# zixunh/vipe

Measured on AMD Instinct MI355X. Metric: dense-BA+flow update iters/s, 512x384 48-KF graph, higher is better.
Workload: dtype f16 (correlation, GRU; fp32 accumulate) + f32 geometry/BA (fp64 reduced system)

## Files before the change

### vipe_amd/csrc/ba.hip

```cpp
#include <stdlib.h>

#include "term_geom.cuh"

namespace {

#include "ba_common.cuh"
#include "ba_plan.inc"
#include "ba_accumulate.inc"
#include "ba_solve_band.inc"
#include "ba_solve_dense.inc"
#include "ba_solve_global.inc"
#include "ba_retract.inc"

hipEvent_t overlap_event() {
  static thread_local hipEvent_t ev[64] = {};
  int d = 0;
  (void)hipGetDevice(&d);
  hipEvent_t& e = ev[d & 63];
  if (!e && hipEventCreateWithFlags(&e, hipEventDisableTiming) != hipSuccess) e = nullptr;
  return e;
}

int overlap_piece(const vipe_ba_params& p, hipEvent_t ev, int piece, int n_pieces, bool gated) {
  hipStream_t side = (hipStream_t)p.overlap_stream;
  if (gated && ev && hipStreamWaitEvent(side, ev, 0) != hipSuccess) return VIPE_EINVAL;
  return p.overlap_fn(p.overlap_user, piece, n_pieces, p.overlap_stream);
}

template <int CAM, int F>
int run_iters(const BAArgs& a, hipStream_t s, int* pieces_done) {
  const int tiles = (a.P + TILE - 1) / TILE;
  const size_t sbytes = sizeof(double) * (size_t)a.w.ld * a.w.ld;
  const size_t nmax = (size_t)a.w.ld - 1;
  const size_t fixed = ((sizeof(SolveLds) + 15) / 16) * 16;
  int panel_cap = (int)std::min<size_t>(nmax + 1, (150 * 1024 - fixed) / (NB * sizeof(double)));
  panel_cap = (panel_cap + 3) & ~3;
  const size_t solve_lds = fixed + (size_t)NB * panel_cap * sizeof(double);
  const size_t band_lds = 158 * 1024;
  static std::atomic<uint64_t> attr_set{0};
  vipe_once_per_device(attr_set, [] {
    (void)hipFuncSetAttribute((const void*)ba_solve_band_kernel, hipFuncAttributeMaxDynamicSharedMemorySize, 160 * 1024);
    (void)hipFuncSetAttribute((const void*)ba_solve_kernel, hipFuncAttributeMaxDynamicSharedMemorySize, 160 * 1024);
    (void)hipFuncSetAttribute((const void*)ba_solve_dense_kernel, hipFuncAttributeMaxDynamicSharedMemorySize, 160 * 1024);
    (void)hipFuncSetAttribute((const void*)chol_backsub_kernel, hipFuncAttributeMaxDynamicSharedMemorySize, 64 * 1024);
  });
  static std::atomic<uint64_t> tmpl_set{0};
  vipe_once_per_device(tmpl_set, [] {
    (void)hipFuncSetAttribute((const void*)ba_accum_mfma_kernel<CAM, F>, hipFuncAttributeMaxDynamicSharedMemorySize, (int)accum_mfma_lds());
    (void)hipFuncSetAttribute((const void*)ba_walk_kernel<CAM, F>, hipFuncAttributeMaxDynamicSharedMemorySize, (int)walk_lds());
    (void)hipFuncSetAttribute((const void*)ba_walk_rig_kernel<CAM, 4>, hipFuncAttributeMaxDynamicSharedMemorySize, (int)walk_rig_lds());
    (void)hipFuncSetAttribute((const void*)ba_walk_rig_kernel<CAM, RG_VMAX>, hipFuncAttributeMaxDynamicSharedMemorySize, (int)walk_rig_lds());
  });
  const bool retract_clears = !a.p.motion_only;
  const bool overlap = a.p.overlap_stream && a.p.overlap_fn;
  hipEvent_t ev = overlap ? overlap_event() : nullptr;
  for (int it = 0; it < a.p.n_iters; ++it) {
    if (!(retract_clears && (it > 0 || a.p.reuse_plan))) {
      hipError_t e1 = hipMemsetAsync(a.w.S, 0, sbytes, s);
      hipError_t e2 = hipMemsetAsync(a.w.Hd, 0, sizeof(double) * nmax, s);
      if (e1 != hipSuccess || e2 != hipSuccess) return (int)(e1 != hipSuccess ? e1 : e2);
    }
    if (a.mv) {
      if (a.p.n_views <= 4) ba_walk_rig_kernel<CAM, 4><<<dim3(tiles, a.nF), TILE, walk_rig_lds(), s>>>(a);
      else ba_walk_rig_kernel<CAM, RG_VMAX><<<dim3(tiles, a.nF), TILE, walk_rig_lds(), s>>>(a);
      ba_schur_kernel<0><<<dim3(SC_GRID, a.nF), TILE, 0, s>>>(a);
      if (ev && hipEventRecord(ev, s) != hipSuccess) return VIPE_EINVAL;
      ba_solve_kernel<<<1, SOLVE_T, solve_lds, s>>>(a, panel_cap);
      launch_tiled_cholesky(a, s);
      if (overlap) {
        const int rc = overlap_piece(a.p, ev, it, a.p.n_iters, true);
        if (rc != VIPE_OK) return rc;
        ++*pieces_done;
      }
      if (!a.p.motion_only) ba_retract_kernel<0><<<dim3(tiles, a.nF), TILE, 0, s>>>(a);
      continue;
    }
    const int hint = a.force_general ? 0 : a.p.path_hint;
    const bool prof = a.p.profile_ev0 && a.p.profile_ev1 &&
                      it == (a.p.profile_iter < 0 || a.p.profile_iter >= a.p.n_iters ? a.p.n_iters - 1 : a.p.profile_iter);
    if (prof && hipEventRecord((hipEvent_t)a.p.profile_ev0, s) != hipSuccess) return VIPE_EINVAL;
    if (!(hint & 2)) ba_accum_mfma_kernel<CAM, F><<<dim3(tiles, a.nF), TILE, accum_mfma_lds(), s>>>(a);
    if (!(hint & 1)) {
      ba_walk_kernel<CAM, F><<<dim3(tiles, a.nF), TILE, walk_lds(), s>>>(a);
      ba_schur_kernel<F><<<dim3(SC_GRID, a.nF), TILE, 0, s>>>(a);
    }
    if (prof && hipEventRecord((hipEvent_t)a.p.profile_ev1, s) != hipSuccess) return VIPE_EINVAL;
    if (ev && hipEventRecord(ev, s) != hipSuccess) return VIPE_EINVAL;
    if (!(hint & 8)) ba_solve_band_kernel<<<1, 2 * BAND_T, band_lds, s>>>(a, (int)(band_lds / sizeof(double)));
    if (!(hint & 16)) ba_solve_dense_kernel<<<1, DN_T, band_lds, s>>>(a, (int)(band_lds / sizeof(double)));
    if (!(hint & 4)) {
      ba_solve_kernel<<<1, SOLVE_T, solve_lds, s>>>(a, panel_cap);
      launch_tiled_cholesky(a, s);
    }
    if (overlap) {
      const int rc = overlap_piece(a.p, ev, it, a.p.n_iters, true);
      if (rc != VIPE_OK) return rc;
      ++*pieces_done;
    }
    if (!a.p.motion_only) ba_retract_kernel<F><<<dim3(tiles, a.nF), TILE, 0, s>>>(a);
  }
  return vipe_launch_status();
}

}

VIPE_EXPORT int64_t vipe_dense_ba_workspace_bytes(const vipe_ba_params* p) {
  if (!p || p->n_poses <= 0 || p->n_views <= 0 || p->ht <= 0 || p->wd <= 0 || p->M < 0) return VIPE_EINVAL;
  return (int64_t)carve(*p, nullptr, nullptr);
}

VIPE_EXPORT int vipe_dense_ba(const vipe_ba_params* p, float* d_poses, float* d_disps, const float* d_disps_sens,
                              float* d_intrinsics, float* d_rig, const float* d_target, const float* d_weight,
                              const float* d_disp_damping, const int64_t* d_pi, const int64_t* d_qi,
                              const int64_t* d_pj, const int64_t* d_qj, const int64_t* d_di, void* d_workspace,
                              int64_t workspace_bytes, int* d_info, void* stream) {
  VIPE_CHECK_ARG(p && d_poses && d_disps && d_disps_sens && d_intrinsics && d_rig && d_disp_damping && d_workspace);
  VIPE_CHECK_ARG(p->n_poses > 0 && p->n_views > 0 && p->ht > 0 && p->wd > 0 && p->M >= 0 && p->n_iters >= 0);
  VIPE_CHECK_ARG(p->t0 <= p->t1 && p->intr_factor > 0);
  VIPE_CHECK_ARG(p->camera == VIPE_CAM_PINHOLE || p->camera == VIPE_CAM_MEI);
  VIPE_CHECK_ARG(p->M == 0 || (d_target && d_weight && d_pi && d_qi && d_pj && d_qj && d_di));
  if (is_multiview(*p) && p->n_views > RG_VMAX) return VIPE_EUNSUPPORTED;
  if ((int64_t)p->n_poses * p->n_views > 65535) return VIPE_EINVAL;
  BAArgs a;
  a.p = *p;
  if ((int64_t)carve(*p, (char*)d_workspace, &a.w) > workspace_bytes) return VIPE_ENOSPACE;
  a.poses = d_poses; a.disps = d_disps; a.intr = d_intrinsics; a.rig = d_rig;
  a.sens = d_disps_sens; a.target = d_target; a.weight = d_weight; a.eta = d_disp_damping;
  a.pi = d_pi; a.qi = d_qi; a.pj = d_pj; a.qj = d_qj; a.di = d_di;
  a.P = p->ht * p->wd;
  a.nF = p->n_poses * p->n_views;
  a.D = p->camera == VIPE_CAM_MEI ? 1 : 0;
  a.mv = is_multiview(*p) ? 1 : 0;
  a.nintr = tail_intr(*p);
  a.ntail = a.nintr + tail_rig(*p);
  a.force_general = (p->solver_options & VIPE_BA_OPT_GENERAL_ACCUMULATE) != 0;
  a.band2 = !(p->solver_options & VIPE_BA_OPT_ONE_CHAIN);
  a.droid = 0;
  a.dz_out = nullptr;
  hipStream_t s = as_stream(stream);
  int rc = VIPE_OK, pieces_done = 0;
  if (p->M > 0 && p->n_iters > 0) {
    ba_sens_kernel<<<a.nF, 256, 0, s>>>(d_disps_sens, a.w.sens_sum, a.P, a.w.info);
    if (!p->reuse_plan) ba_plan_kernel<<<1, 1024, 0, s>>>(a);
    const int F = p->optimize_intrinsics ? 1 + a.D : 0;
    if (p->camera == VIPE_CAM_PINHOLE) rc = F ? run_iters<VIPE_CAM_PINHOLE, 1>(a, s, &pieces_done) : run_iters<VIPE_CAM_PINHOLE, 0>(a, s, &pieces_done);
    else rc = F ? run_iters<VIPE_CAM_MEI, 2>(a, s, &pieces_done) : run_iters<VIPE_CAM_MEI, 0>(a, s, &pieces_done);
    if (rc != VIPE_OK) return rc;
    if (d_info) {
      hipError_t e = hipMemcpyAsync(d_info, a.w.info, 8 * sizeof(int), hipMemcpyDeviceToDevice, s);
      if (e != hipSuccess) return (int)e;
    }
  }
  if (p->overlap_stream && p->overlap_fn) {
    const int n_pieces = p->n_iters > 0 ? p->n_iters : 1;
    for (; pieces_done < n_pieces; ++pieces_done) {
      rc = overlap_piece(*p, nullptr, pieces_done, n_pieces, false);
      if (rc != VIPE_OK) return rc;
    }
  }
  const int64_t nd = (int64_t)a.nF * a.P;
  clamp_min_kernel<<<(int)std::min<int64_t>((nd + 255) / 256, 2048), 256, 0, s>>>(d_disps, nd, 1e-3f);
  return vipe_launch_status();
}

namespace {
size_t droid_extra_bytes(int E) { return align_up(8 * (size_t)(E + 1)) + align_up(7 * 4); }
vipe_ba_params droid_params(int n_poses, int ht, int wd, int E, int t0, int t1, int iterations, float lm, float ep,
                            int motion_only) {
  vipe_ba_params p = {};
  p.n_poses = n_poses; p.n_views = 1; p.ht = ht; p.wd = wd; p.M = E; p.t0 = t0; p.t1 = t1; p.n_iters = iterations;
  p.pose_damping = lm; p.pose_ep = ep; p.motion_only = motion_only; p.limited_disp = 0; p.optimize_intrinsics = 0;
  p.optimize_rig_rotation = 0; p.camera = VIPE_CAM_PINHOLE; p.alpha = 0.05f; p.weight_scale = 0.001f; p.intr_factor = 1.0f;
  p.reuse_plan = 0; p.path_hint = 0;
  return p;
}
}

VIPE_EXPORT int64_t vipe_ba_workspace_bytes(int n_poses, int ht, int wd, int E) {
  if (n_poses <= 0 || ht <= 0 || wd <= 0 || E < 0) return VIPE_EINVAL;
  const vipe_ba_params p = droid_params(n_poses, ht, wd, E, 0, 0, 0, 0.f, 0.f, 0);
  return (int64_t)(carve(p, nullptr, nullptr) + droid_extra_bytes(E));
}

VIPE_EXPORT int vipe_ba(float* d_poses, float* d_disps, const float* d_intrinsics, const float* d_disps_sens,
                        const float* d_targets, const float* d_weights, const float* d_eta, const int64_t* d_ii,
                        const int64_t* d_jj, int n_poses, int ht, int wd, int E, int n_eta, int t0, int t1,
                        int iterations, float lm, float ep, int motion_only, float* d_dx, float* d_dz,
                        void* d_workspace, int64_t workspace_bytes, void* stream) {
  VIPE_CHECK_ARG(d_poses && d_disps && d_intrinsics && d_disps_sens && d_eta && d_workspace && d_dx && d_dz);
  VIPE_CHECK_ARG(n_poses > 0 && ht > 0 && wd > 0 && E >= 0 && iterations >= 0 && n_eta >= 0);
  VIPE_CHECK_ARG(0 <= t0 && t0 <= t1 && t1 <= n_poses);
  VIPE_CHECK_ARG(E == 0 || (d_targets && d_weights && d_ii && d_jj));
  if (n_poses > 65535) return VIPE_EINVAL;
  BAArgs a;
  a.p = droid_params(n_poses, ht, wd, E, t0, t1, iterations, lm, ep, motion_only);
  const size_t base = carve(a.p, (char*)d_workspace, &a.w);
  if ((int64_t)(base + droid_extra_bytes(E)) > workspace_bytes) return VIPE_ENOSPACE;
  int64_t* zeros = (int64_t*)((char*)d_workspace + base);
  float* rig = (float*)((char*)d_workspace + base + align_up(8 * (size_t)(E + 1)));
  hipStream_t s = as_stream(stream);
  const float rig_id[7] = {0, 0, 0, 0, 0, 0, 1};
  hipError_t e0 = hipMemsetAsync(zeros, 0, 8 * (size_t)(E + 1), s);
  hipError_t e1 = hipMemcpyAsync(rig, rig_id, sizeof(rig_id), hipMemcpyHostToDevice, s);
  const int64_t P = (int64_t)ht * wd;
  hipError_t e2 = hipMemsetAsync(d_dx, 0, sizeof(float) * 6 * (size_t)(t1 - t0), s);
  hipError_t e3 = hipMemsetAsync(d_dz, 0, sizeof(float) * (size_t)n_eta * P, s);
  if (e0 != hipSuccess || e1 != hipSuccess || e2 != hipSuccess || e3 != hipSuccess) return VIPE_EINVAL;
  a.poses = d_poses; a.disps = d_disps; a.intr = (float*)d_intrinsics; a.rig = rig;
  a.sens = d_disps_sens; a.target = d_targets; a.weight = d_weights; a.eta = d_eta;
  a.pi = d_ii; a.qi = zeros; a.pj = d_jj; a.qj = zeros; a.di = d_ii;
  a.P = ht * wd; a.nF = n_poses; a.D = 0;
  a.mv = 0; a.nintr = 0; a.ntail = 0;
  a.force_general = 0;
  a.band2 = 1;
  a.droid = 1;
  a.dz_out = d_dz;
  if (iterations == 0 || t1 == t0) return VIPE_OK;
  ba_sens_kernel<<<a.nF, 256, 0, s>>>(d_disps_sens, a.w.sens_sum, a.P, a.w.info);
  ba_plan_kernel<<<1, 1024, 0, s>>>(a);
  int pieces_done = 0;
  const int rc = run_iters<VIPE_CAM_PINHOLE, 0>(a, s, &pieces_done);
  if (rc != VIPE_OK) return rc;
  hipError_t e4 = hipMemcpyAsync(d_dx, a.w.dx, sizeof(float) * 6 * (size_t)(t1 - t0), hipMemcpyDeviceToDevice, s);
  return e4 == hipSuccess ? vipe_launch_status() : (int)e4;
}
```

### vipe_amd/csrc/ba_accumulate.inc

```
constexpr int AM_ROWS = 48;
constexpr int AM_P1 = 130;
constexpr int AM_P2 = 66;
constexpr int AM_P2H = 34;
constexpr int AM_WBUF = 16 * AM_P1;
static_assert(AM_ROWS * AM_P2H <= AM_WBUF, "R2 half image must fit the wave buffer");
constexpr int AM_SP = AM_ROWS + 1;

struct TermGeomM {
  TermGeom g;
  float Mi[36];
};

constexpr size_t accum_mfma_lds() {
  return sizeof(float) * (NWAVE * AM_WBUF + AM_ROWS * AM_SP + AM_DMAX * 256 + 64) + AM_DMAX * sizeof(TermGeomM);
}

typedef float float4m __attribute__((ext_vector_type(4)));


__device__ __forceinline__ void term_setup_m(const BAArgs& a, int e, TermGeomM& m) {
  TermGeom& g = m.g;
  term_setup(a, e, g);
#pragma unroll
  for (int c = 0; c < 6; ++c) {
    float ec[6] = {0, 0, 0, 0, 0, 0}, col[6];
    ec[c] = 1.0f;
    adjT_apply(g.G, ec, col);
#pragma unroll
    for (int r = 0; r < 6; ++r) m.Mi[r * 6 + c] = (g.merge == 1 && r == c ? 1.0f : 0.0f) - col[r];
  }
}

template <int F>
struct WalkPixel {
  static constexpr int FF = F > 0 ? F : 1;
  int p;
  bool inb;
  float d, X0, Y0, dX0[FF], dY0[FF];
  float C, wz, Ei[6], Efr[FF];
};

template <int CAM, int F>
__device__ __forceinline__ WalkPixel<F> walk_pixel(const BAArgs& a, int k, int qi) {
  WalkPixel<F> px;
  const int p_raw = blockIdx.x * TILE + threadIdx.x;
  px.inb = p_raw < a.P;
  px.p = px.inb ? p_raw : a.P - 1;
  const cam::Intr Ii = cam::load_scaled(a.intr + qi * (4 + a.D), a.D, 1.0f / a.p.intr_factor);
  const float u = (float)(px.p % a.p.wd), v = (float)(px.p / a.p.wd);
  px.d = a.disps[(int64_t)k * a.P + px.p];
  cam::iproj<CAM, F>(Ii, u, v, px.X0, px.Y0, px.dX0, px.dY0);
  px.C = px.wz = 0.f;
#pragma unroll
  for (int q = 0; q < 6; ++q) px.Ei[q] = 0.f;
#pragma unroll
  for (int f = 0; f < px.FF; ++f) px.Efr[f] = 0.f;
  return px;
}

template <int CAM, int F>
__device__ __forceinline__ void term_point_jacobians(const TermGeom& G, const WalkPixel<F>& px, float& Z, float& x, float& y,
                                                     float (&Jp)[2][3], float (&Jfj)[2][WalkPixel<F>::FF], float (&Ja)[3][6]) {
  const float X0 = px.X0, Y0 = px.Y0, d = px.d;
  const float X = G.T.R[0] * X0 + G.T.R[1] * Y0 + G.T.R[2] + G.T.t[0] * d;
  const float Y = G.T.R[3] * X0 + G.T.R[4] * Y0 + G.T.R[5] + G.T.t[1] * d;
  Z = G.T.R[6] * X0 + G.T.R[7] * Y0 + G.T.R[8] + G.T.t[2] * d;
  cam::proj<CAM, true, F>(G.Ij, X, Y, Z, x, y, Jp, Jfj);
  const float J0[3][6] = {{d, 0, 0, 0, Z, -Y}, {0, d, 0, -Z, 0, X}, {0, 0, d, Y, -X, 0}};
#pragma unroll
  for (int r = 0; r < 3; ++r) {
#pragma unroll
    for (int q = 0; q < 6; ++q) Ja[r][q] = J0[r][q];
  }
  if (G.rig_adj) {
#pragma unroll
    for (int r = 0; r < 3; ++r) {
      float tmp[6];
      adjT_apply(G.Rr, Ja[r], tmp);
#pragma unroll
      for (int q = 0; q < 6; ++q) Ja[r][q] = tmp[q];
    }
  }
}

__device__ __forceinline__ void term_row_jacobians(const float (&Jpc)[3], const float (&Ja)[3][6], const Rigid& T,
                                                   float (&Jj)[6], float& Jz) {
#pragma unroll
  for (int q = 0; q < 6; ++q) Jj[q] = Jpc[0] * Ja[0][q] + Jpc[1] * Ja[1][q] + Jpc[2] * Ja[2][q];
  Jz = Jpc[0] * T.t[0] + Jpc[1] * T.t[1] + Jpc[2] * T.t[2];
}

__device__ __forceinline__ float term_row_src_intr(const float (&Jpc)[3], const Rigid& T, float dX0, float dY0) {
  const float ax = T.R[0] * dX0 + T.R[1] * dY0;
  const float ay = T.R[3] * dX0 + T.R[4] * dY0;
  const float az = T.R[6] * dX0 + T.R[7] * dY0;
  return Jpc[0] * ax + Jpc[1] * ay + Jpc[2] * az;
}

__device__ __forceinline__ float4m gram_r1(const float* wbuf, int l16, int kq) {
  __builtin_amdgcn_fence(__ATOMIC_RELEASE, "wavefront");
  __builtin_amdgcn_wave_barrier();
  float4m g4 = {0.f, 0.f, 0.f, 0.f};
  const float* arow = wbuf + l16 * AM_P1 + kq;
#pragma unroll 8
  for (int s = 0; s < 32; ++s) {
    const float av = arow[4 * s];
    g4 = __builtin_amdgcn_mfma_f32_16x16x4f32(av, av, g4, 0, 0, 0);
  }
  return g4;
}

template <int CAM, int F>
__device__ __forceinline__ void walk_tile(const BAArgs& a, const TermGeomM* tg, int deg, bool dfree, float* wbuf,
                                          float* acc1, WalkPixel<F>& px) {
  constexpr int FF = F > 0 ? F : 1;
  constexpr int RPT = F > 0 ? 16 : 8;
  constexpr int TPT = 16 / RPT;
  const BAWs& w = a.w;
  const int P = a.P, p = px.p, lane = threadIdx.x & 63, l16 = lane & 15, kq = lane >> 4;
  const bool inb = px.inb;
  float2 nx_t[TPT], nx_w[TPT];
  auto prefetch = [&](int t0) {
#pragma unroll
    for (int uu = 0; uu < TPT; ++uu) {
      const int t = min(t0 + uu, deg - 1);
      load_tw(a, tg[t].g.e, p, P, nx_t[uu], nx_w[uu]);
    }
  };
  prefetch(0);
  for (int t0 = 0; t0 < deg; t0 += TPT) {
    float2 cur_t[TPT], cur_w[TPT];
#pragma unroll
    for (int uu = 0; uu < TPT; ++uu) { cur_t[uu] = nx_t[uu]; cur_w[uu] = nx_w[uu]; }
    if (t0 + TPT < deg) prefetch(t0 + TPT);
#pragma unroll
    for (int uu = 0; uu < TPT; ++uu) {
      const int t = t0 + uu;
      if (t >= deg) break;
      const TermGeom& G = tg[t].g;
      const int e = G.e;
      float Z, x, y, Jp[2][3], Jfj[2][FF], Ja[3][6];
      term_point_jacobians<CAM, F>(G, px, Z, x, y, Jp, Jfj, Ja);
      const float2 tgt = cur_t[uu], wg = cur_w[uu];
      const float val = valid_weight(a, Z, inb);
      const float wd2[2] = {val * wg.x, val * wg.y};
      const float wc[2] = {G.merge == 2 ? 0.0f : wd2[0], G.merge == 2 ? 0.0f : wd2[1]};
      const float rc[2] = {x - tgt.x, y - tgt.y};
      const bool fj = G.sj >= 0;
      float Ejv[6] = {0, 0, 0, 0, 0, 0};
#pragma unroll
      for (int c = 0; c < 2; ++c) {
        float Jj[6], Ji[6], Jf[FF], Jz;
        term_row_jacobians(Jp[c], Ja, G.T, Jj, Jz);
        if constexpr (F > 0) {
#pragma unroll
          for (int f = 0; f < F; ++f)
            Jf[f] = (term_row_src_intr(Jp[c], G.T, px.dX0[f], px.dY0[f]) + Jfj[c][f]) * (1.0f / a.p.intr_factor);
        }
        const float sw = __builtin_amdgcn_sqrtf(wc[c]);
        float* col = wbuf + (uu * RPT) * AM_P1 + c * 64 + lane;
#pragma unroll
        for (int q = 0; q < 6; ++q) col[q * AM_P1] = Jj[q] * sw;
        col[6 * AM_P1] = rc[c] * sw;
        if constexpr (F > 0) {
#pragma unroll
          for (int f = 0; f < F; ++f) col[(7 + f) * AM_P1] = Jf[f] * sw;
        }
        if (dfree) {
          const float wJz = wc[c] * Jz;
          px.C += wd2[c] * Jz * Jz;
          px.wz -= wd2[c] * Jz * rc[c];
          float tmp[6];
          adjT_apply(G.G, Jj, tmp);
#pragma unroll
          for (int q = 0; q < 6; ++q) {
            Ji[q] = (G.merge == 1 ? Jj[q] : 0.0f) - tmp[q];
            px.Ei[q] += Ji[q] * wJz;
          }
          if constexpr (F > 0) {
#pragma unroll
            for (int f = 0; f < F; ++f) px.Efr[f] += Jf[f] * wJz;
          }
#pragma unroll
          for (int q = 0; q < 6; ++q) Ejv[q] += Jj[q] * wJz;
        }
      }
      if (dfree && fj && inb) {
#pragma unroll
        for (int q = 0; q < 6; ++q) w.Ej[((int64_t)e * 6 + q) * P + p] = Ejv[q];
      }
    }
    const float4m g4 = gram_r1(wbuf, l16, kq);
#pragma unroll
    for (int r = 0; r < 4; ++r) {
      const int row = 4 * kq + r;
      const int tb = row / RPT;
      if (l16 / RPT == tb && t0 + tb < deg) atomicAdd(&acc1[(t0 + tb) * 256 + (row % RPT) * 16 + (l16 % RPT)], g4[r]);
    }
    __builtin_amdgcn_wave_barrier();
  }
}

template <int F>
__device__ __forceinline__ void flush_term_blocks(const BAWs& w, const TermGeomM* tg, int deg, const float* acc1, float* accI,
                                                  float* T1 , int si, int nrow, int foff) {
  constexpr int FF = F > 0 ? F : 1;
  const int lane = threadIdx.x & 63, wave = threadIdx.x >> 6;
  const bool fi = si >= 0;
  for (int t = wave; t < deg; t += NWAVE) {
    const TermGeomM& TG = tg[t];
    const float* Gm = acc1 + t * 256;
    const float* Mi = TG.Mi;
    const int sj = TG.g.sj;
    const bool fj = sj >= 0;
    const int bj = 6 * sj, bi = 6 * si;
    if (lane < 36) {
      const int r = lane / 6, c = lane % 6;
      const float hjj = Gm[r * 16 + c];
      if (fj && r >= c) {
        s_add(w, bj + r, bj + c, (double)hjj);
        if (r == c) atomicAdd(&w.Hd[bj + r], (double)hjj);
      }
      float t1 = 0.f;
#pragma unroll
      for (int q = 0; q < 6; ++q) t1 += Mi[r * 6 + q] * Gm[q * 16 + c];
      T1[r * 8 + c] = t1;
      if (fi && fj) s_add(w, bi + r, bj + c, (double)t1);
    } else if (lane < 42) {
      const int q = lane - 36;
      const float vjn = Gm[q * 16 + 6];
      if (fj) atomicAdd(&w.S[(int64_t)nrow * w.ld + bj + q], -(double)vjn);
      if (fi) {
        float vin = 0.f;
#pragma unroll
        for (int c = 0; c < 6; ++c) vin += Mi[q * 6 + c] * Gm[c * 16 + 6];
        atomicAdd(&accI[36 + q], -vin);
      }
    } else if (F > 0 && lane < 42 + 6 * F) {
      const int q = (lane - 42) / FF, f = (lane - 42) % FF;
      const float hjf = Gm[q * 16 + 7 + f];
      if (fj) s_add(w, foff + f, bj + q, (double)hjf);
      if (fi) {
        float hif = 0.f;
#pragma unroll
        for (int c = 0; c < 6; ++c) hif += Mi[q * 6 + c] * Gm[c * 16 + 7 + f];
        atomicAdd(&accI[42 + q * FF + f], hif);
      }
    } else if (F > 0 && lane < 42 + 6 * F + F * F) {
      const int i2 = lane - 42 - 6 * F, f = i2 / FF, f2 = i2 % FF;
      if (f >= f2) atomicAdd(&accI[42 + 6 * FF + f * FF + f2], Gm[(7 + f) * 16 + 7 + f2]);
    } else if (F > 0 && lane < 42 + 6 * F + F * F + F) {
      const int f = lane - 42 - 6 * F - F * F;
      atomicAdd(&accI[42 + 6 * FF + FF * FF + f], -Gm[(7 + f) * 16 + 6]);
    }
    __builtin_amdgcn_fence(__ATOMIC_RELEASE, "wavefront");
    __builtin_amdgcn_wave_barrier();
    if (fi && lane < 36) {
      const int r = lane / 6, c = lane % 6;
      float hii = 0.f;
#pragma unroll
      for (int q = 0; q < 6; ++q) hii += T1[r * 8 + q] * Mi[c * 6 + q];
      atomicAdd(&accI[r * 6 + c], hii);
    }
    __builtin_amdgcn_wave_barrier();
  }
}

template <int F>
__device__ __forceinline__ void flush_frame_blocks(const BAWs& w, const float* accI, int si, int nrow, int foff) {
  constexpr int FF = F > 0 ? F : 1;
  const int tid = threadIdx.x;
  const bool fi = si >= 0;
  const int bi = 6 * si;
  if (tid < 36) {
    const int r = tid / 6, c = tid % 6;
    if (fi && r >= c) {
      const double s = (double)accI[r * 6 + c];
      s_add(w, bi + r, bi + c, s);
      if (r == c) atomicAdd(&w.Hd[bi + r], s);
    }
  } else if (tid < 42) {
    if (fi) atomicAdd(&w.S[(int64_t)nrow * w.ld + bi + (tid - 36)], (double)accI[tid]);
  } else if (F > 0 && tid < 42 + 6 * F) {
    const int q = (tid - 42) / FF, f = (tid - 42) % FF;
    if (fi) s_add(w, foff + f, bi + q, (double)accI[tid]);
  } else if (F > 0 && tid < 42 + 6 * F + F * F) {
    const int i2 = tid - 42 - 6 * F, f = i2 / FF, f2 = i2 % FF;
    if (f >= f2) {
      const double s = (double)accI[tid];
      s_add(w, foff + f, foff + f2, s);
      if (f == f2) atomicAdd(&w.Hd[foff + f], s);
    }
  } else if (F > 0 && tid < 42 + 6 * F + F * F + F) {
    atomicAdd(&w.S[(int64_t)nrow * w.ld + foff + (tid - 42 - 6 * F - F * F)], (double)accI[tid]);
  }
}

template <int NF, int F>
__device__ __forceinline__ void store_disp_block(const BAArgs& a, int k, int flags, WalkPixel<F>& px) {
  static_assert(NF <= WalkPixel<F>::FF, "E_f rows come from px.Efr");
  const BAWs& w = a.w;
  const int P = a.P, p = px.p;
  const int64_t kp = (int64_t)k * P + p;
  finish_disp(a, k, p, P, flags, px.d, px.C, px.wz);
  if (px.inb) {
    w.C[kp] = px.C;
    w.wv[kp] = px.wz;
#pragma unroll
    for (int q = 0; q < 6; ++q) w.Ekk[((int64_t)k * 6 + q) * P + p] = px.Ei[q];
#pragma unroll
    for (int f = 0; f < NF; ++f) w.Ef[((int64_t)k * 2 + f) * P + p] = px.Efr[f];
  }
}

template <int CAM, int F>
__global__ __launch_bounds__(TILE) __attribute__((amdgpu_waves_per_eu(3, 3))) void ba_accum_mfma_kernel(BAArgs a) {
  const vipe_ba_params& prm = a.p;
  const BAWs& w = a.w;
  if (a.force_general || w.info[6] > AM_DMAX) return;
  const int k = blockIdx.y;
  const int beg = w.rowptr[k], end = w.rowptr[k + 1];
  if (beg == end) return;
  const int deg = end - beg;
  const int P = a.P, V = prm.n_views, tid = threadIdx.x, lane = tid & 63, wave = tid >> 6;
  const int flags = w.fflags[k];
  const bool dfree = flags & 2;
  const int pose_i = k / V, qi = k % V;
  const int si = w.pose_slot[pose_i];
  const bool fi = si >= 0;
  const int n_free = w.info[0], nrow = w.info[3];
  const int foff = 6 * n_free;

  extern __shared__ __align__(16) float am_smem[];
  float* wbuf = am_smem + wave * AM_WBUF;
  float* accS = am_smem + NWAVE * AM_WBUF;
  float* acc1 = accS + AM_ROWS * AM_SP;
  float* accI = acc1 + AM_DMAX * 256;
  TermGeomM* tg = reinterpret_cast<TermGeomM*>(accI + 64);

  for (int i = tid; i < AM_ROWS * AM_SP + AM_DMAX * 256 + 64; i += TILE) accS[i] = 0.0f;
  if (tid < deg) {
    TermGeomM m;
    term_setup_m(a, w.order[beg + tid], m);
    tg[tid] = m;
  }
  __syncthreads();

  WalkPixel<F> px = walk_pixel<CAM, F>(a, k, qi);
  const int l16 = lane & 15, kq = lane >> 4;
  walk_tile<CAM, F>(a, tg, deg, dfree, wbuf, acc1, px);

  const int NR = 6 * (deg + 1) + F + 1;
  if (dfree) {
    store_disp_block<F>(a, k, flags, px);
    const float sq = px.inb ? __builtin_amdgcn_rsqf(px.C) : 0.0f;
    float ej[AM_DMAX][6];
#pragma unroll
    for (int t = 0; t < AM_DMAX; ++t) {
      const bool on = t < deg && tg[min(t, deg - 1)].g.sj >= 0 && px.inb;
      const int64_t eb = (int64_t)tg[min(t, deg - 1)].g.e * 6 * P + px.p;
#pragma unroll
      for (int q = 0; q < 6; ++q) ej[t][q] = on ? w.Ej[eb + (int64_t)q * P] : 0.0f;
    }
    constexpr int NPAIR = 6;
    float4m g4[NPAIR];
#pragma unroll
    for (int i = 0; i < NPAIR; ++i) g4[i] = float4m{0.f, 0.f, 0.f, 0.f};
    const int RT = (NR + 15) >> 4;
#pragma unroll
    for (int half = 0; half < 2; ++half) {
      if ((lane >> 5) == half) {
        float* col = wbuf + (lane & 31);
#pragma unroll
        for (int q = 0; q < 6; ++q) col[q * AM_P2H] = fi ? px.Ei[q] * sq : 0.0f;
#pragma unroll
        for (int t = 0; t < AM_DMAX; ++t) {
          if (t < deg) {
#pragma unroll
            for (int q = 0; q < 6; ++q) col[(6 * (t + 1) + q) * AM_P2H] = ej[t][q] * sq;
          }
        }
        if constexpr (F > 0) {
#pragma unroll
          for (int f = 0; f < F; ++f) col[(6 * (deg + 1) + f) * AM_P2H] = px.Efr[f] * sq;
        }
        col[(NR - 1) * AM_P2H] = px.wz * sq;
        for (int r = NR; r < ((NR + 15) & ~15); ++r) col[r * AM_P2H] = 0.0f;
      }
      __builtin_amdgcn_fence(__ATOMIC_RELEASE, "wavefront");
      __builtin_amdgcn_wave_barrier();
#pragma unroll
      for (int ta = 0; ta < 3; ++ta)
#pragma unroll
        for (int tb = 0; tb <= ta; ++tb) {
          if (ta < RT) {
            const float* ar = wbuf + (16 * ta + l16) * AM_P2H + kq;
            const float* br = wbuf + (16 * tb + l16) * AM_P2H + kq;
            float4m acc = g4[ta * (ta + 1) / 2 + tb];
#pragma unroll
            for (int s = 0; s < 8; ++s) acc = __builtin_amdgcn_mfma_f32_16x16x4f32(ar[4 * s], br[4 * s], acc, 0, 0, 0);
            g4[ta * (ta + 1) / 2 + tb] = acc;
          }
        }
      __builtin_amdgcn_fence(__ATOMIC_RELEASE, "wavefront");
      __builtin_amdgcn_wave_barrier();
    }
#pragma unroll
    for (int ta = 0; ta < 3; ++ta)
#pragma unroll
      for (int tb = 0; tb <= ta; ++tb) {
        if (ta < RT) {
#pragma unroll
          for (int r = 0; r < 4; ++r) {
            const int row = 16 * ta + 4 * kq + r, cc = 16 * tb + l16;
            if (row < NR && cc <= row) atomicAdd(&accS[row * AM_SP + cc], g4[ta * (ta + 1) / 2 + tb][r]);
          }
        }
      }
  }
  __syncthreads();

  flush_term_blocks<F>(w, tg, deg, acc1, accI, wbuf, si, nrow, foff);
  __syncthreads();

  flush_frame_blocks<F>(w, accI, si, nrow, foff);
  if (dfree) {
    auto gmap = [&](int row) -> int {
      if (row >= 6 * (deg + 1)) return foff + (row - 6 * (deg + 1));
      const int m = row / 6, q = row % 6;
      const int sl = m == 0 ? si : tg[m - 1].g.sj;
      return sl >= 0 ? 6 * sl + q : -1;
    };
    for (int i = tid; i < NR * NR; i += TILE) {
      const int row = i / NR, cc = i % NR;
      if (cc > row || cc == NR - 1) continue;
      const int gc = gmap(cc);
      if (gc < 0) continue;
      const float val = accS[row * AM_SP + cc];
      if (row == NR - 1) {
        atomicAdd(&w.S[(int64_t)nrow * w.ld + gc], -(double)val);
      } else {
        const int gr = gmap(row);
        if (gr >= 0) s_add(w, gr, gc, (gr == gc && row != cc) ? -2.0 * (double)val : -(double)val);
      }
    }
  }
}

constexpr int WK_CH = 8;
constexpr int WK_CH1 = 12;
constexpr size_t walk_lds() {
  return sizeof(float) * (NWAVE * 16 * AM_P1 + WK_CH1 * 256 + 64) + WK_CH1 * sizeof(TermGeomM);
}

template <int CAM, int F>
__global__ __launch_bounds__(TILE) void ba_walk_kernel(BAArgs a) {
  constexpr int WBUF = 16 * AM_P1;
  const vipe_ba_params& prm = a.p;
  const BAWs& w = a.w;
  if (!a.force_general && w.info[6] <= AM_DMAX) return;
  const int k = blockIdx.y;
  const int beg = w.rowptr[k], end = w.rowptr[k + 1];
  if (beg == end) return;
  const int deg_all = end - beg;
  const int V = prm.n_views, tid = threadIdx.x, wave = tid >> 6;
  const int flags = w.fflags[k];
  const bool dfree = flags & 2;
  const int pose_i = k / V, qi = k % V;
  const int si = w.pose_slot[pose_i];
  const int n_free = w.info[0], nrow = w.info[3];
  const int foff = 6 * n_free;

  extern __shared__ __align__(16) float am_smem[];
  float* wbuf = am_smem + wave * WBUF;
  float* acc1 = am_smem + NWAVE * WBUF;
  float* accI = acc1 + WK_CH1 * 256;
  TermGeomM* tg = reinterpret_cast<TermGeomM*>(accI + 64);
  if (tid < 64) accI[tid] = 0.0f;

  WalkPixel<F> px = walk_pixel<CAM, F>(a, k, qi);

  for (int cb = 0; cb < deg_all; cb += WK_CH1) {
    const int deg = min(WK_CH1, deg_all - cb);
    __syncthreads();
    for (int i = tid; i < WK_CH1 * 256; i += TILE) acc1[i] = 0.0f;
    if (tid < deg) {
      TermGeomM m;
      term_setup_m(a, w.order[beg + cb + tid], m);
      tg[tid] = m;
    }
    __syncthreads();

    walk_tile<CAM, F>(a, tg, deg, dfree, wbuf, acc1, px);

    __syncthreads();
    flush_term_blocks<F>(w, tg, deg, acc1, accI, wbuf, si, nrow, foff);

  }
  __syncthreads();

  flush_frame_blocks<F>(w, accI, si, nrow, foff);
  if (dfree) store_disp_block<F>(a, k, flags, px);
}

constexpr int RG_NB = 10;
constexpr int RG_NL = 28;
struct TermGeomR {
  TermGeom g;
  int qj, same_view;
  int gcol[RG_NL];
  float Lm[RG_NL][RG_NB];
};
constexpr size_t walk_rig_lds() {
  return sizeof(float) * (NWAVE * 16 * AM_P1 + WK_CH * 256) + WK_CH * sizeof(TermGeomR);
}
__device__ __forceinline__ int rg_tile_row(int b) { return b < 6 ? b : b + 1; }

template <int CAM, int VM>
__global__ __launch_bounds__(TILE) void ba_walk_rig_kernel(BAArgs a) {
  constexpr int WBUF = 16 * AM_P1;
  constexpr int F = CAM == VIPE_CAM_MEI ? 2 : 1;
  const vipe_ba_params& prm = a.p;
  const BAWs& w = a.w;
  const int k = blockIdx.y;
  const int beg = w.rowptr[k], end = w.rowptr[k + 1];
  if (beg == end) return;
  const int deg_all = end - beg;
  const int P = a.P, V = prm.n_views, tid = threadIdx.x, lane = tid & 63, wave = tid >> 6;
  const int flags = w.fflags[k];
  const bool dfree = flags & 2;
  const int pose_i = k / V, qi = k % V;
  const int si = w.pose_slot[pose_i];
  const int n_free = w.info[0], nrow = w.info[3];
  const int foff = 6 * n_free, roff = foff + a.nintr;
  const bool oi = prm.optimize_intrinsics, orr = prm.optimize_rig_rotation;

  extern __shared__ __align__(16) float am_smem[];
  float* wbuf = am_smem + wave * WBUF;
  float* acc1 = am_smem + NWAVE * WBUF;
  TermGeomR* tg = reinterpret_cast<TermGeomR*>(acc1 + WK_CH * 256);

  WalkPixel<F> px = walk_pixel<CAM, F>(a, k, qi);
  const int p = px.p;
  const bool inb = px.inb;
  float ErA[6] = {0, 0, 0, 0, 0, 0};
  float Efv[VM][F] = {}, Erv[VM][6] = {};
  const int l16 = lane & 15, kq = lane >> 4;

  for (int cb = 0; cb < deg_all; cb += WK_CH) {
    const int deg = min(WK_CH, deg_all - cb);
    __syncthreads();
    for (int i = tid; i < WK_CH * 256; i += TILE) acc1[i] = 0.0f;
    if (tid < deg) {
      TermGeomR& m = tg[tid];
      const int e = w.order[beg + cb + tid];
      const int pi = (int)a.pi[e], pj = (int)a.pj[e], qj = (int)a.qj[e];
      term_transforms(a.poses, a.rig, pi, qi, pj, qj, m.g.T, m.g.G, m.g.Rr);
      m.g.Ij = cam::load_scaled(a.intr + qj * (4 + a.D), a.D, 1.0f / prm.intr_factor);
      m.g.e = e;
      m.g.merge = (pi == pj);
      m.g.rig_adj = !(m.g.Rr.t[0] == 0.f && m.g.Rr.t[1] == 0.f && m.g.Rr.t[2] == 0.f && m.g.Rr.R[0] == 1.f &&
                      m.g.Rr.R[4] == 1.f && m.g.Rr.R[8] == 1.f);
      m.g.sj = m.g.merge ? -1 : w.pose_slot[pj];
      m.qj = qj;
      m.same_view = (qj == qi);
      const int sjj = w.pose_slot[pj];
      for (int c = 0; c < RG_NL; ++c)
        for (int b = 0; b < RG_NB; ++b) m.Lm[c][b] = 0.0f;
      for (int c = 0; c < 6; ++c) {
        float ec[6] = {0, 0, 0, 0, 0, 0}, col[6];
        ec[c] = 1.0f;
        adjT_apply(m.g.G, ec, col);
        for (int r = 0; r < 6; ++r) {
          m.Lm[r][c] = -col[r];
          m.Lm[16 + r][c] = col[r];
        }
        m.Lm[6 + c][c] = 1.0f;
        m.Lm[22 + c][c] = -1.0f;
      }
      for (int f = 0; f < 2; ++f) {
        m.Lm[12 + f][6 + f] = 1.0f;
        m.Lm[14 + f][8 + f] = 1.0f;
      }
      for (int q = 0; q < 6; ++q) {
        m.gcol[q] = si >= 0 ? 6 * si + q : -1;
        m.gcol[6 + q] = sjj >= 0 ? 6 * sjj + q : -1;
        m.gcol[16 + q] = (orr && qi >= 1) ? roff + 6 * (qi - 1) + q : -1;
        m.gcol[22 + q] = (orr && qj >= 1) ? roff + 6 * (qj - 1) + q : -1;
      }
      for (int f = 0; f < 2; ++f) {
        m.gcol[12 + f] = (oi && f < F) ? foff + qi * F + f : -1;
        m.gcol[14 + f] = (oi && f < F && qj != qi) ? foff + qj * F + f : -1;
      }
    }
    __syncthreads();

    for (int t = 0; t < deg; ++t) {
      const TermGeom& G = tg[t].g;
      const int e = G.e, qj = tg[t].qj;
      const bool same = tg[t].same_view;
      float Z, x, y, Jp[2][3], Jfj[2][F], Ja[3][6];
      term_point_jacobians<CAM, F>(G, px, Z, x, y, Jp, Jfj, Ja);
      float2 tgt, wg;
      load_tw(a, e, p, P, tgt, wg);
      const float val = valid_weight(a, Z, inb);
      const float wc[2] = {val * wg.x, val * wg.y};
      const float rc[2] = {x - tgt.x, y - tgt.y};
      float Ejv[6] = {0, 0, 0, 0, 0, 0};
#pragma unroll
      for (int c = 0; c < 2; ++c) {
        float Jj[6], JfA[F], JfB[F], Jz;
        term_row_jacobians(Jp[c], Ja, G.T, Jj, Jz);
#pragma unroll
        for (int f = 0; f < F; ++f) {
          const float ji = term_row_src_intr(Jp[c], G.T, px.dX0[f], px.dY0[f]) * (1.0f / prm.intr_factor);
          const float jj = Jfj[c][f] * (1.0f / prm.intr_factor);
          JfA[f] = same ? ji + jj : ji;
          JfB[f] = same ? 0.0f : jj;
        }
        const float sw = __builtin_amdgcn_sqrtf(wc[c]);
        float* col = wbuf + c * 64 + lane;
#pragma unroll
        for (int q = 0; q < 6; ++q) col[q * AM_P1] = Jj[q] * sw;
        col[6 * AM_P1] = rc[c] * sw;
#pragma unroll
        for (int f = 0; f < 2; ++f) {
          col[(7 + f) * AM_P1] = f < F ? JfA[f < F ? f : 0] * sw : 0.0f;
          col[(9 + f) * AM_P1] = f < F ? JfB[f < F ? f : 0] * sw : 0.0f;
        }
#pragma unroll
        for (int r = 11; r < 16; ++r) col[r * AM_P1] = 0.0f;
        if (dfree) {
// ... 204 lines not shown
```

### vipe_amd/csrc/ba_common.cuh

```cuda

constexpr int TILE = 256;
constexpr int NWAVE = TILE / WAVE;
constexpr int TCHUNK = 8;
constexpr int AM_DMAX = 6;

struct BAWs {
  int* rowptr;
  int* order;
  int* pose_slot;
  int* slot_pose;
  int* fflags;
  int* scratch;
  int* info;
  float* sens_sum;
  float* C;
  float* wv;
  float* Ekk;
  float* Ef;
  float* Et;
  float* Ej;
  double* S;
  double* Hd;
  float* dx;
  double* Wi;
  int* krow;
  int ld;
};

struct BAArgs {
  vipe_ba_params p;
  float *poses, *disps, *intr, *rig;
  const float *sens, *target, *weight, *eta;
  const int64_t *pi, *qi, *pj, *qj, *di;
  BAWs w;
  int P, nF, D;
  int mv, nintr, ntail;
  int force_general;
  int band2;
  int droid;
  float* dz_out;
};

inline size_t align_up(size_t x, size_t a = 256) { return (x + a - 1) / a * a; }

constexpr int RG_VMAX = 8;
inline bool is_multiview(const vipe_ba_params& p) { return p.n_views > 1; }
inline int tail_intr(const vipe_ba_params& p) {
  const int F = 1 + (p.camera == VIPE_CAM_MEI ? 1 : 0);
  return p.optimize_intrinsics ? (is_multiview(p) ? p.n_views * F : F) : 0;
}
inline int tail_rig(const vipe_ba_params& p) { return p.optimize_rig_rotation ? 6 * (p.n_views - 1) : 0; }

size_t carve(const vipe_ba_params& p, char* base, BAWs* out) {
  const size_t nP = p.n_poses, nF = (size_t)p.n_poses * p.n_views, P = (size_t)p.ht * p.wd, M = p.M;
  const size_t ntail_max = is_multiview(p) ? (size_t)p.n_views * 2 + 6 * (size_t)(p.n_views - 1) : 2;
  const size_t nmax = 6 * nP + ntail_max;
  size_t off = 0;
  auto take = [&](size_t bytes) {
    char* ptr = base ? base + off : nullptr;
    off += align_up(bytes);
    return ptr;
  };
  BAWs w;
  w.rowptr = (int*)take(4 * (nF + 1));
  w.order = (int*)take(4 * (M + 1));
  w.pose_slot = (int*)take(4 * nP);
  w.slot_pose = (int*)take(4 * nP);
  w.fflags = (int*)take(4 * nF);
  w.scratch = (int*)take(4 * (2 * nP + nF));
  w.info = (int*)take(4 * 8);
  w.sens_sum = (float*)take(4 * nF);
  w.C = (float*)take(4 * nF * P);
  w.wv = (float*)take(4 * nF * P);
  w.Ekk = (float*)take(4 * nF * 6 * P);
  w.Ef = (float*)take(4 * nF * 2 * P);
  w.Et = (float*)take(is_multiview(p) ? 4 * nF * ntail_max * P : 0);
  w.Ej = (float*)take(4 * (M + 1) * 6 * P);
  w.S = (double*)take(8 * (nmax + 1) * (nmax + 1));
  w.Hd = (double*)take(8 * (nmax + 16));
  w.dx = (float*)take(4 * nmax);
  w.Wi = (double*)take(8 * 64 * 64 * ((nmax + 63) / 64));
  w.krow = (int*)take(4 * (nF + 1));
  w.ld = (int)(nmax + 1);
  if (out) *out = w;
  return off;
}

__device__ __forceinline__ void load_tw(const BAArgs& a, int e, int p, int P, float2& tgt, float2& wg) {
  if (a.droid) {
    const int64_t o = (int64_t)e * 2 * P + p;
    tgt = make_float2(a.target[o], a.target[o + P]);
    wg = make_float2(a.weight[o], a.weight[o + P]);
  } else {
    const int64_t o2 = ((int64_t)e * P + p) * 2;
    tgt = *reinterpret_cast<const float2*>(a.target + o2);
    wg = *reinterpret_cast<const float2*>(a.weight + o2);
  }
}
__device__ __forceinline__ float valid_weight(const BAArgs& a, float Z, bool inb) {
  const bool ok = a.droid ? !(Z < 0.25f) : (Z > cam::MIN_DEPTH);
  return (inb && ok) ? a.p.weight_scale : 0.0f;
}
__device__ __forceinline__ void term_setup(const BAArgs& a, int e, TermGeom& g) {
  const int pi = (int)a.pi[e], pj = (int)a.pj[e], qj = (int)a.qj[e];
  term_transforms(a.poses, a.rig, pi, (int)a.qi[e], pj, qj, g.T, g.G, g.Rr);
  g.Ij = cam::load_scaled(a.intr + qj * (4 + a.D), a.D, 1.0f / a.p.intr_factor);
  g.e = e;
  g.merge = (pi == pj);
  if (a.droid && pi == pj) {
    g.merge = 2;
    for (int i = 0; i < 9; ++i) g.T.R[i] = g.G.R[i] = (i % 4 == 0) ? 1.0f : 0.0f;
    g.T.t[0] = g.G.t[0] = -0.1f;
    g.T.t[1] = g.T.t[2] = g.G.t[1] = g.G.t[2] = 0.0f;
  }
  g.rig_adj = !(g.Rr.t[0] == 0.f && g.Rr.t[1] == 0.f && g.Rr.t[2] == 0.f && g.Rr.R[0] == 1.f &&
                g.Rr.R[4] == 1.f && g.Rr.R[8] == 1.f);
  g.sj = g.merge ? -1 : a.w.pose_slot[pj];
}
__device__ __forceinline__ void finish_disp(const BAArgs& a, int k, int p, int P, int flags, float d, float& C, float& wz) {
  const int64_t kp = (int64_t)k * P + p;
  if (a.droid) {
    const float sv = a.sens[kp];
    if (sv > 0.0f) { C += a.p.alpha; wz -= a.p.alpha * (d - sv); }
    else C += a.eta[(int64_t)a.w.krow[k] * P + p];
  } else {
    if (a.w.sens_sum[k] > 0.0f) {
      C += a.p.alpha;
      wz -= a.p.alpha * (d - a.sens[kp]);
    }
    C += 1e-7f + (0.2f * a.eta[kp] + 1e-7f);
  }
}

__device__ __forceinline__ void s_add(const BAWs& w, int row, int col, double v) {
  if (row < col) { int tmp = row; row = col; col = tmp; }
  atomicAdd(&w.S[(int64_t)row * w.ld + col], v);
}

__device__ __forceinline__ double rsqrt_nr(double x) {
  double r = __builtin_amdgcn_rsq(x);
  const double hx = 0.5 * x;
  r = r * __builtin_fma(-hx * r, r, 1.5);
  r = r * __builtin_fma(-hx * r, r, 1.5);
  return r;
}
```

### vipe_amd/csrc/ba_retract.inc

```

template <int F>
__global__ __launch_bounds__(TILE) void ba_retract_kernel(BAArgs a) {
  const BAWs& w = a.w;
  {
    const int64_t nthr = (int64_t)gridDim.x * gridDim.y * TILE;
    const int64_t gid = ((int64_t)blockIdx.y * gridDim.x + blockIdx.x) * TILE + threadIdx.x;
    const int64_t ns = (int64_t)w.ld * w.ld;
    for (int64_t i = gid; i < ns; i += nthr) w.S[i] = 0.0;
    for (int64_t i = gid; i < (int64_t)w.ld - 1; i += nthr) w.Hd[i] = 0.0;
  }
  const int k = blockIdx.y;
  const int flags = w.fflags[k];
  if (!(flags & 2)) return;
  const int P = a.P, V = a.p.n_views;
  const int p = blockIdx.x * TILE + threadIdx.x;
  if (p >= P) return;
  const int64_t kp = (int64_t)k * P + p;
  if (flags & 8) {
    float C = 0.f, wz = 0.f;
    finish_disp(a, k, p, P, flags, a.disps[kp], C, wz);
    const float dz = wz / C;
    a.disps[kp] += dz;
    if (a.dz_out) a.dz_out[(int64_t)w.krow[k] * P + p] = dz;
    return;
  }
  const int beg = w.rowptr[k], end = w.rowptr[k + 1];
  float rhs = w.wv[kp];
  const int si = w.pose_slot[k / V];
  const int n_free = w.info[0];
  const int smin = a.droid ? 1 : 0;
  if (si >= smin) {
#pragma unroll
    for (int q = 0; q < 6; ++q) rhs -= w.Ekk[((int64_t)k * 6 + q) * P + p] * w.dx[6 * si + q];
  }
  for (int c = beg; c < end; ++c) {
    const int e = w.order[c];
    const int pj = (int)a.pj[e];
    const int sj = ((int)a.pi[e] == pj) ? -1 : w.pose_slot[pj];
    if (sj < smin) continue;
#pragma unroll
    for (int q = 0; q < 6; ++q) rhs -= w.Ej[((int64_t)e * 6 + q) * P + p] * w.dx[6 * sj + q];
  }
  if constexpr (F > 0) {
#pragma unroll
    for (int f = 0; f < F; ++f) rhs -= w.Ef[((int64_t)k * 2 + f) * P + p] * w.dx[6 * n_free + f];
  }
  if (a.mv) {
    for (int f = 0; f < a.ntail; ++f) rhs -= w.Et[((int64_t)k * a.ntail + f) * P + p] * w.dx[6 * n_free + f];
  }
  float dz = rhs / w.C[kp];
  if (!a.droid && dz > 10.0f) dz = 0.0f;
  a.disps[kp] += dz;
  if (a.dz_out) a.dz_out[(int64_t)w.krow[k] * P + p] = dz;
}

__global__ void clamp_min_kernel(float* __restrict__ x, int64_t n, float lo) {
  for (int64_t i = (int64_t)blockIdx.x * blockDim.x + threadIdx.x; i < n; i += (int64_t)gridDim.x * blockDim.x)
    x[i] = fmaxf(x[i], lo);
}
```

Measured before the change: 271.2.

## Fuse disparity retraction into next iteration's accumulate prologue with double-buffered S

Except on the last iteration, the per-iteration retract kernel is dropped. The disparity update now runs in the prologue of the next iteration's accumulate and walk kernels. The reduced system S/Hd is ping-ponged between two buffers so the other buffer can be cleared inside the same launch. The final disparity clamp is folded into the last retract kernel, which removes one more launch and one more pass over memory. The cost is a second S buffer in the workspace, redundant clears in both prologue kernels, and a correctness dependence on whichever accumulate kernel runs each iteration doing the retraction.

```diff
diff --git a/vipe_amd/csrc/ba.hip b/vipe_amd/csrc/ba.hip
--- a/vipe_amd/csrc/ba.hip
+++ b/vipe_amd/csrc/ba.hip
@@ -1,4 +1,6 @@
 #include <stdlib.h>
+
+#include <utility>
 
 #include "term_geom.cuh"
 
@@ -28,10 +30,10 @@
 }
 
 template <int CAM, int F>
-int run_iters(const BAArgs& a, hipStream_t s, int* pieces_done) {
-  const int tiles = (a.P + TILE - 1) / TILE;
-  const size_t sbytes = sizeof(double) * (size_t)a.w.ld * a.w.ld;
-  const size_t nmax = (size_t)a.w.ld - 1;
+int run_iters(const BAArgs& a0, hipStream_t s, int* pieces_done) {
+  const int tiles = (a0.P + TILE - 1) / TILE;
+  const size_t sbytes = sizeof(double) * (size_t)a0.w.ld * a0.w.ld;
+  const size_t nmax = (size_t)a0.w.ld - 1;
   const size_t fixed = ((sizeof(SolveLds) + 15) / 16) * 16;
   int panel_cap = (int)std::min<size_t>(nmax + 1, (150 * 1024 - fixed) / (NB * sizeof(double)));
   panel_cap = (panel_cap + 3) & ~3;
@@ -51,10 +53,19 @@
     (void)hipFuncSetAttribute((const void*)ba_walk_rig_kernel<CAM, 4>, hipFuncAttributeMaxDynamicSharedMemorySize, (int)walk_rig_lds());
     (void)hipFuncSetAttribute((const void*)ba_walk_rig_kernel<CAM, RG_VMAX>, hipFuncAttributeMaxDynamicSharedMemorySize, (int)walk_rig_lds());
   });
-  const bool retract_clears = !a.p.motion_only;
-  const bool overlap = a.p.overlap_stream && a.p.overlap_fn;
+  const bool retract_clears = !a0.p.motion_only;
+  const bool fused = retract_clears && !a0.mv;
+  const int last = a0.p.n_iters - 1;
+  const bool overlap = a0.p.overlap_stream && a0.p.overlap_fn;
   hipEvent_t ev = overlap ? overlap_event() : nullptr;
-  for (int it = 0; it < a.p.n_iters; ++it) {
+  for (int it = 0; it < a0.p.n_iters; ++it) {
+    BAArgs a = a0;
+    if (fused && (it & 1)) {
+      std::swap(a.w.S, a.w.S_alt);
+      std::swap(a.w.Hd, a.w.Hd_alt);
+    }
+    a.pre = fused ? ((it > 0 ? 1 : 0) | (it < last ? 2 : 0)) : 0;
+    a.clamp = a0.clamp && it == last;
     if (!(retract_clears && (it > 0 || a.p.reuse_plan))) {
       hipError_t e1 = hipMemsetAsync(a.w.S, 0, sbytes, s);
       hipError_t e2 = hipMemsetAsync(a.w.Hd, 0, sizeof(double) * nmax, s);
@@ -97,7 +108,7 @@
       if (rc != VIPE_OK) return rc;
       ++*pieces_done;
     }
-    if (!a.p.motion_only) ba_retract_kernel<F><<<dim3(tiles, a.nF), TILE, 0, s>>>(a);
+    if (!a.p.motion_only && it == last) ba_retract_kernel<F><<<dim3(tiles, a.nF), TILE, 0, s>>>(a);
   }
   return vipe_launch_status();
 }
@@ -137,6 +148,9 @@
   a.band2 = !(p->solver_options & VIPE_BA_OPT_ONE_CHAIN);
   a.droid = 0;
   a.dz_out = nullptr;
+  a.pre = 0;
+  const bool retract_clamps = p->M > 0 && p->n_iters > 0 && !p->motion_only;
+  a.clamp = retract_clamps ? 1 : 0;
   hipStream_t s = as_stream(stream);
   int rc = VIPE_OK, pieces_done = 0;
   if (p->M > 0 && p->n_iters > 0) {
@@ -158,8 +172,10 @@
       if (rc != VIPE_OK) return rc;
     }
   }
-  const int64_t nd = (int64_t)a.nF * a.P;
-  clamp_min_kernel<<<(int)std::min<int64_t>((nd + 255) / 256, 2048), 256, 0, s>>>(d_disps, nd, 1e-3f);
+  if (!retract_clamps) {
+    const int64_t nd = (int64_t)a.nF * a.P;
+    clamp_min_kernel<<<(int)std::min<int64_t>((nd + 255) / 256, 2048), 256, 0, s>>>(d_disps, nd, 1e-3f);
+  }
   return vipe_launch_status();
 }
 
@@ -215,6 +231,8 @@
   a.band2 = 1;
   a.droid = 1;
   a.dz_out = d_dz;
+  a.pre = 0;
+  a.clamp = 0;
   if (iterations == 0 || t1 == t0) return VIPE_OK;
   ba_sens_kernel<<<a.nF, 256, 0, s>>>(d_disps_sens, a.w.sens_sum, a.P, a.w.info);
   ba_plan_kernel<<<1, 1024, 0, s>>>(a);
diff --git a/vipe_amd/csrc/ba_accumulate.inc b/vipe_amd/csrc/ba_accumulate.inc
--- a/vipe_amd/csrc/ba_accumulate.inc
+++ b/vipe_amd/csrc/ba_accumulate.inc
@@ -56,6 +56,56 @@
 #pragma unroll
   for (int f = 0; f < px.FF; ++f) px.Efr[f] = 0.f;
   return px;
+}
+
+template <int F>
+__device__ __forceinline__ float retract_pixel(const BAArgs& a, int k, int p, int flags) {
+  const BAWs& w = a.w;
+  const int P = a.P, V = a.p.n_views;
+  const int64_t kp = (int64_t)k * P + p;
+  if (flags & 8) {
+    float C = 0.f, wz = 0.f;
+    const float d0 = a.disps[kp];
+    finish_disp(a, k, p, P, flags, d0, C, wz);
+    const float dz = wz / C;
+    if (a.dz_out) a.dz_out[(int64_t)w.krow[k] * P + p] = dz;
+    return d0 + dz;
+  }
+  const int beg = w.rowptr[k], end = w.rowptr[k + 1];
+  float rhs = w.wv[kp];
+  const int si = w.pose_slot[k / V];
+  const int n_free = w.info[0];
+  const int smin = a.droid ? 1 : 0;
+  if (si >= smin) {
+#pragma unroll
+    for (int q = 0; q < 6; ++q) rhs -= w.Ekk[((int64_t)k * 6 + q) * P + p] * w.dx[6 * si + q];
+  }
+  for (int c = beg; c < end; ++c) {
+    const int e = w.order[c];
+    const int pj = (int)a.pj[e];
+    const int sj = ((int)a.pi[e] == pj) ? -1 : w.pose_slot[pj];
+    if (sj < smin) continue;
+#pragma unroll
+    for (int q = 0; q < 6; ++q) rhs -= w.Ej[((int64_t)e * 6 + q) * P + p] * w.dx[6 * sj + q];
+  }
+  if constexpr (F > 0) {
+#pragma unroll
+    for (int f = 0; f < F; ++f) rhs -= w.Ef[((int64_t)k * 2 + f) * P + p] * w.dx[6 * n_free + f];
+  }
+  if (a.mv) {
+    for (int f = 0; f < a.ntail; ++f) rhs -= w.Et[((int64_t)k * a.ntail + f) * P + p] * w.dx[6 * n_free + f];
+  }
+  float dz = rhs / w.C[kp];
+  if (!a.droid && dz > 10.0f) dz = 0.0f;
+  if (a.dz_out) a.dz_out[(int64_t)w.krow[k] * P + p] = dz;
+  return a.disps[kp] + dz;
+}
+
+template <int F>
+__device__ __forceinline__ void accum_prologue(const BAArgs& a, int k, int flags) {
+  if (a.pre & 2) clear_reduced(a.w.S_alt, a.w.Hd_alt, a.w.ld);
+  const int p = blockIdx.x * TILE + threadIdx.x;
+  if ((a.pre & 1) && (flags & 2) && p < a.P) a.disps[(int64_t)k * a.P + p] = retract_pixel<F>(a, k, p, flags);
 }
 
 template <int CAM, int F>
@@ -319,11 +369,12 @@
   const BAWs& w = a.w;
   if (a.force_general || w.info[6] > AM_DMAX) return;
   const int k = blockIdx.y;
+  const int flags = w.fflags[k];
+  accum_prologue<F>(a, k, flags);
   const int beg = w.rowptr[k], end = w.rowptr[k + 1];
   if (beg == end) return;
   const int deg = end - beg;
   const int P = a.P, V = prm.n_views, tid = threadIdx.x, lane = tid & 63, wave = tid >> 6;
-  const int flags = w.fflags[k];
   const bool dfree = flags & 2;
   const int pose_i = k / V, qi = k % V;
   const int si = w.pose_slot[pose_i];
@@ -460,11 +511,12 @@
   const BAWs& w = a.w;
   if (!a.force_general && w.info[6] <= AM_DMAX) return;
   const int k = blockIdx.y;
+  const int flags = w.fflags[k];
+  accum_prologue<F>(a, k, flags);
   const int beg = w.rowptr[k], end = w.rowptr[k + 1];
   if (beg == end) return;
   const int deg_all = end - beg;
   const int V = prm.n_views, tid = threadIdx.x, wave = tid >> 6;
-  const int flags = w.fflags[k];
   const bool dfree = flags & 2;
   const int pose_i = k / V, qi = k % V;
   const int si = w.pose_slot[pose_i];
@@ -478,6 +530,7 @@
   TermGeomM* tg = reinterpret_cast<TermGeomM*>(accI + 64);
   if (tid < 64) accI[tid] = 0.0f;
 
+  if (a.pre & 1) __syncthreads();
   WalkPixel<F> px = walk_pixel<CAM, F>(a, k, qi);
 
   for (int cb = 0; cb < deg_all; cb += WK_CH1) {
diff --git a/vipe_amd/csrc/ba_common.cuh b/vipe_amd/csrc/ba_common.cuh
--- a/vipe_amd/csrc/ba_common.cuh
+++ b/vipe_amd/csrc/ba_common.cuh
@@ -21,6 +21,8 @@
   float* Ej;
   double* S;
   double* Hd;
+  double* S_alt;
+  double* Hd_alt;
   float* dx;
   double* Wi;
   int* krow;
@@ -39,6 +41,8 @@
   int band2;
   int droid;
   float* dz_out;
+  int pre;
+  int clamp;
 };
 
 inline size_t align_up(size_t x, size_t a = 256) { return (x + a - 1) / a * a; }
@@ -78,6 +82,8 @@
   w.Ej = (float*)take(4 * (M + 1) * 6 * P);
   w.S = (double*)take(8 * (nmax + 1) * (nmax + 1));
   w.Hd = (double*)take(8 * (nmax + 16));
+  w.S_alt = (double*)take(8 * (nmax + 1) * (nmax + 1));
+  w.Hd_alt = (double*)take(8 * (nmax + 16));
   w.dx = (float*)take(4 * nmax);
   w.Wi = (double*)take(8 * 64 * 64 * ((nmax + 63) / 64));
   w.krow = (int*)take(4 * (nF + 1));
@@ -137,6 +143,14 @@
   atomicAdd(&w.S[(int64_t)row * w.ld + col], v);
 }
 
+__device__ __forceinline__ void clear_reduced(double* S, double* Hd, int ld) {
+  const int64_t nthr = (int64_t)gridDim.x * gridDim.y * TILE;
+  const int64_t gid = ((int64_t)blockIdx.y * gridDim.x + blockIdx.x) * TILE + threadIdx.x;
+  const int64_t ns = (int64_t)ld * ld;
+  for (int64_t i = gid; i < ns; i += nthr) S[i] = 0.0;
+  for (int64_t i = gid; i < (int64_t)ld - 1; i += nthr) Hd[i] = 0.0;
+}
+
 __device__ __forceinline__ double rsqrt_nr(double x) {
   double r = __builtin_amdgcn_rsq(x);
   const double hx = 0.5 * x;
diff --git a/vipe_amd/csrc/ba_retract.inc b/vipe_amd/csrc/ba_retract.inc
--- a/vipe_amd/csrc/ba_retract.inc
+++ b/vipe_amd/csrc/ba_retract.inc
@@ -2,56 +2,16 @@
 template <int F>
 __global__ __launch_bounds__(TILE) void ba_retract_kernel(BAArgs a) {
   const BAWs& w = a.w;
-  {
-    const int64_t nthr = (int64_t)gridDim.x * gridDim.y * TILE;
-    const int64_t gid = ((int64_t)blockIdx.y * gridDim.x + blockIdx.x) * TILE + threadIdx.x;
-    const int64_t ns = (int64_t)w.ld * w.ld;
-    for (int64_t i = gid; i < ns; i += nthr) w.S[i] = 0.0;
-    for (int64_t i = gid; i < (int64_t)w.ld - 1; i += nthr) w.Hd[i] = 0.0;
-  }
+  clear_reduced(w.S, w.Hd, w.ld);
+  clear_reduced(w.S_alt, w.Hd_alt, w.ld);
   const int k = blockIdx.y;
   const int flags = w.fflags[k];
-  if (!(flags & 2)) return;
-  const int P = a.P, V = a.p.n_views;
   const int p = blockIdx.x * TILE + threadIdx.x;
-  if (p >= P) return;
-  const int64_t kp = (int64_t)k * P + p;
-  if (flags & 8) {
-    float C = 0.f, wz = 0.f;
-    finish_disp(a, k, p, P, flags, a.disps[kp], C, wz);
-    const float dz = wz / C;
-    a.disps[kp] += dz;
-    if (a.dz_out) a.dz_out[(int64_t)w.krow[k] * P + p] = dz;
-    return;
-  }
-  const int beg = w.rowptr[k], end = w.rowptr[k + 1];
-  float rhs = w.wv[kp];
-  const int si = w.pose_slot[k / V];
-  const int n_free = w.info[0];
-  const int smin = a.droid ? 1 : 0;
-  if (si >= smin) {
-#pragma unroll
-    for (int q = 0; q < 6; ++q) rhs -= w.Ekk[((int64_t)k * 6 + q) * P + p] * w.dx[6 * si + q];
-  }
-  for (int c = beg; c < end; ++c) {
-    const int e = w.order[c];
-    const int pj = (int)a.pj[e];
-    const int sj = ((int)a.pi[e] == pj) ? -1 : w.pose_slot[pj];
-    if (sj < smin) continue;
-#pragma unroll
-    for (int q = 0; q < 6; ++q) rhs -= w.Ej[((int64_t)e * 6 + q) * P + p] * w.dx[6 * sj + q];
-  }
-  if constexpr (F > 0) {
-#pragma unroll
-    for (int f = 0; f < F; ++f) rhs -= w.Ef[((int64_t)k * 2 + f) * P + p] * w.dx[6 * n_free + f];
-  }
-  if (a.mv) {
-    for (int f = 0; f < a.ntail; ++f) rhs -= w.Et[((int64_t)k * a.ntail + f) * P + p] * w.dx[6 * n_free + f];
-  }
-  float dz = rhs / w.C[kp];
-  if (!a.droid && dz > 10.0f) dz = 0.0f;
-  a.disps[kp] += dz;
-  if (a.dz_out) a.dz_out[(int64_t)w.krow[k] * P + p] = dz;
+  if (p >= a.P || !((flags & 2) || a.clamp)) return;
+  const int64_t kp = (int64_t)k * a.P + p;
+  float d = (flags & 2) ? retract_pixel<F>(a, k, p, flags) : a.disps[kp];
+  if (a.clamp) d = fmaxf(d, 1e-3f);
+  a.disps[kp] = d;
 }
 
 __global__ void clamp_min_kernel(float* __restrict__ x, int64_t n, float lo) {
```

Result: no change. 270.2 (-0.4%).
